# NOAA-GFDL/icebergs

Hardware: AMD Instinct MI355X
Metric: berg_steps_per_sec (higher is better)
Workload: dtype f64; 1 GPU; BASELINE configs[4] per-GPU share with configs[1] physics: 10000000 synthetic bergs/GPU (random mass classes), 360x200 lat-lon ocean grid, RK4 drag+Coriolis+melt+mass spreading, dt=1800 s, ignore_traj=T; bergs_per_gpu=10000000, grid=360x200, exchange=none (1 GPU), bergs_alive_at_end=9999583

## Files before the change

icebergs_amd/csrc/kid_cells.inc:

```
#include "kid_planes.hpp"

namespace {
struct GridPlanes { const double *st[KID_NGRID_STATIC]; const double *fo[KID_NFORCING]; };

__global__ void __launch_bounds__(256) pack_static_kernel(GridPlanes gp, GeoRec *geo, double *hotok, double *latref, double pi_180, int ni, int nj, int latlon, double Lx) {
  const int c = blockIdx.x * 256 + threadIdx.x;
  if (c >= ni * nj) return;
  GeoRec r;
  r.lon = gp.st[KID_G_LON][c]; r.lat = gp.st[KID_G_LAT][c]; r.area = gp.st[KID_G_AREA][c]; r.msk = gp.st[KID_G_MSK][c];
  geo[c] = r;
  if (latref) { double s_, c_; sincos(r.lat * pi_180, &s_, &c_); latref[2 * c] = s_; latref[2 * c + 1] = c_; }
  const int il = c % ni, jl = c / ni;
  double ok = 0.;
  if (il >= 1 && jl >= 1 && il + 1 < ni && jl + 1 < nj) {
    const double *lon = gp.st[KID_G_LON], *lat = gp.st[KID_G_LAT];
    const double x0 = lon[c - ni - 1], y0 = lat[c - ni - 1];
    const double x1 = mod_around(lon[c - ni], x0, Lx), y1 = lat[c - ni];
    const double x2 = mod_around(lon[c], x0, Lx), y2 = lat[c];
    const double x3 = mod_around(lon[c - 1], x0, Lx), y3 = lat[c - 1];
    const double k0 = (x1 - x0) * (y2 - y1) - (y1 - y0) * (x2 - x1), k1 = (x2 - x1) * (y3 - y2) - (y2 - y1) * (x3 - x2);
    const double k2 = (x3 - x2) * (y0 - y3) - (y3 - y2) * (x0 - x3), k3 = (x0 - x3) * (y1 - y0) - (y0 - y3) * (x1 - x0);
    const bool convex = (k0 > 0. && k1 > 0. && k2 > 0. && k3 > 0.) || (k0 < 0. && k1 < 0. && k2 < 0. && k3 < 0.);
    const bool polar = latlon && dmax(dmax(y0, y1), dmax(y2, y3)) >= 89.999;
    const double *lo = gp.st[KID_G_LON];
    const bool rect = lo[c - 1] == lo[c - ni - 1] && lo[c] == lo[c - ni] && lat[c - ni] == lat[c - ni - 1] && lat[c] == lat[c - 1];
    if (convex && !polar) ok = rect ? 2. : 1.;
  }
  hotok[c] = ok;
}

enum { KID_PKT_CELLS_PER_WAVE = 32 };
__global__ void __launch_bounds__(256) pack_packets_kernel(const DevGrid g, double *__restrict__ pkt) {
  const int lane = (int)(threadIdx.x & 63), wave = (int)(threadIdx.x >> 6);
  const int j = (int)blockIdx.y;
  const int i0 = ((int)blockIdx.x * 4 + wave) * KID_PKT_CELLS_PER_WAVE;
  if (i0 >= g.ni) return;
  const bool second = lane < PK_SIZE - 64;
  const PacketSrc s0 = packet_source(g, lane), s1 = packet_source(g, second ? 64 + lane : 0);
  const bool row_inside = j >= 1 && j < g.nj - 1;
  const int i1 = min(i0 + KID_PKT_CELLS_PER_WAVE, g.ni);
  for (int ib = i0; ib < i1; ib += 8) {
    double a[8], a2[8];
#pragma unroll
    for (int u = 0; u < 8; ++u) {
      const int i = ib + u;
      const bool interior = row_inside && i >= 1 && i < g.ni - 1 && i < i1;
      const long long c = interior ? (long long)j * g.ni + i : (long long)g.ni + 1;
      a[u] = *reinterpret_cast<const double *>(s0.base + c * s0.stride);
      a2[u] = *reinterpret_cast<const double *>(s1.base + c * s1.stride);
    }
#pragma unroll
    for (int u = 0; u < 8; ++u) {
      const int i = ib + u;
      if (i >= i1) continue;
      const bool interior = row_inside && i >= 1 && i < g.ni - 1;
      const bool is_cos = lane < PK_CORNER && (lane & 7) == 0, is_sin = lane < PK_CORNER && (lane & 7) == 1;
      const bool rotated = __ballot((is_cos && a[u] != 1.) || (is_sin && a[u] != 0.)) != 0ull;
      const bool nan_stencil = __ballot(lane >= PK_DDX && lane < PK_AREA && a[u] != a[u]) != 0ull;
      double *o = pkt + ((long long)j * g.ni + i) * PK_GSTRIDE;
      o[lane] = interior ? a[u] : 0.;
      if (second) {
        double v = interior ? a2[u] : 0.;
        if (64 + lane == PK_HOTOK) v = interior ? ((v != 0. && !nan_stencil) ? 1. : -1.) * (1. + (v == 2. ? 2. : 0.) + (rotated ? 0. : 4.)) : 0.;
        o[64 + lane] = v;
      }
    }
  }
}

struct PrepExtras { double *ssh_copy; double *acc; int zero_planes; int *cnt0, *cnt1; };
__global__ void __launch_bounds__(256) pack_forcing_kernel(GridPlanes gp, VelRec *vel, TrcRec *trc, int ni, int nj, PrepExtras ex) {
  const int c = blockIdx.x * 256 + threadIdx.x;
  if (c >= ni * nj) return;
  if (ex.ssh_copy) ex.ssh_copy[c] = gp.fo[KID_F_SSH][c];
  if (ex.acc) {
    const size_t ncell = (size_t)ni * (size_t)nj;
    for (int q = 0; q < ex.zero_planes; ++q) ex.acc[(size_t)q * ncell + (size_t)c] = 0.;
  }
  if (c == 0) { if (ex.cnt0) *ex.cnt0 = 0; if (ex.cnt1) *ex.cnt1 = 0; }
  const int il = c % ni, jl = c / ni;
  VelRec v;
  v.cosr = gp.st[KID_G_COS][c]; v.sinr = gp.st[KID_G_SIN][c];
  v.uo = gp.fo[KID_F_UO][c]; v.vo = gp.fo[KID_F_VO][c]; v.ui = gp.fo[KID_F_UI][c]; v.vi = gp.fo[KID_F_VI][c];
  v.ua = gp.fo[KID_F_UA][c]; v.va = gp.fo[KID_F_VA][c];
  vel[c] = v;
  const double *dx = gp.st[KID_G_DX], *dy = gp.st[KID_G_DY], *msk = gp.st[KID_G_MSK], *ssh = gp.fo[KID_F_SSH];
  TrcRec t;
  t.sst = gp.fo[KID_F_SST][c]; t.sss = gp.fo[KID_F_SSS][c]; t.cn = gp.fo[KID_F_CN][c]; t.hi = gp.fo[KID_F_HI][c];
  t.od = gp.st[KID_G_OCEAN_DEPTH][c] + ssh[c];
  t.msk = msk[c];
  t.ddx = 0.; t.ddy = 0.;
  if (il + 1 < ni && jl >= 1) {
    const double dxp = 0.5 * (dx[c + 1] + dx[c + 1 - ni]);
    const double dx0 = 0.5 * (dx[c] + dx[c - ni]);
    t.ddx = 2. * (ssh[c + 1] - ssh[c]) / (dx0 + dxp) * msk[c + 1] * msk[c];
  }
  if (jl + 1 < nj && il >= 1) {
    const double dyp = 0.5 * (dy[c + ni] + dy[c + ni - 1]);
    const double dy0 = 0.5 * (dy[c] + dy[c - 1]);
    t.ddy = 2. * (ssh[c + ni] - ssh[c]) / (dy0 + dyp) * msk[c + ni] * msk[c];
  }
  trc[c] = t;
}

__global__ void set_grid_kernel(const DevGrid src, DevGrid *dst) { if (threadIdx.x == 0 && blockIdx.x == 0) *dst = src; }

__device__ __forceinline__ double nine_point(const DevGrid &g, const double *v, const size_t ncell, const int c, const int i, const bool wrap, const double a, const double m) {
  const int nic = g.iec - g.isc + 1, ni = g.ni;
  const int wm = (wrap && i == g.isc) ? nic : 0, wp = (wrap && i == g.iec) ? -nic : 0;
  double dmda = nine_point_sum([&](int di, int dj, int slot) { return v[(size_t)(slot - 1) * ncell + (size_t)(c + di + (di < 0 ? wm : (di > 0 ? wp : 0)) + dj * ni)]; });
  if (a > 0) dmda = dmda / a * m;
  return dmda;
}

__global__ void __launch_bounds__(256) gather_kernel(const DevGrid g, const kid_params p, double *__restrict__ acc,
                                                     double *__restrict__ out, const size_t ncell, double *__restrict__ totals,
                                                     const double *__restrict__ spread_mass_old, const double *__restrict__ spread_mass_tmp) {
  const int t = blockIdx.x * 256 + threadIdx.x;
  if (t < KID_NSCALAR) {
    totals[t] += (acc - KID_NSCALAR)[t];
    (acc - KID_NSCALAR)[t] = 0.;
  }
  const int nic = g.iec - g.isc + 1, njc = g.jec - g.jsc + 1;
  if (t >= nic * njc) return;
  const int i = g.isc + t % nic, j = g.jsc + t / nic;
  const int c = g.idx(i, j);
  const double a = g.geo[c].area, m = g.geo[c].msk;
  const int dm = p.diag_mask;
  const bool wrap = p.periodic_reentry != 0 && g.Lx > 0.;
  auto nine = [&](int base) { return nine_point(g, acc + (size_t)base * ncell, ncell, c, i, wrap, a, m); };
  double su = 0., sv = 0., sa = 0.;
  if ((dm & KID_DIAG_SPREAD_UVEL) || p.pass_fields_to_ocean_model) su = nine(KID_A_UVEL_ON_OCEAN);
  if ((dm & KID_DIAG_SPREAD_VVEL) || p.pass_fields_to_ocean_model) sv = nine(KID_A_VVEL_ON_OCEAN);
  if ((dm & KID_DIAG_SPREAD_AREA) || p.pass_fields_to_ocean_model) sa = dmin(nine(KID_A_AREA_ON_OCEAN), 1.0);
  const double sm = nine(KID_A_MASS_ON_OCEAN);
  out[(size_t)KID_O_SPREAD_MASS * ncell + c] = sm;
  out[(size_t)KID_O_SPREAD_AREA * ncell + c] = sa;
  out[(size_t)KID_O_SPREAD_UVEL * ncell + c] = su;
  out[(size_t)KID_O_SPREAD_VVEL * ncell + c] = sv;
  if ((dm & KID_DIAG_U_ICEBERG) || (dm & KID_DIAG_V_ICEBERG)) {
    const double mass = acc[(size_t)KID_A_MASS * ncell + c];
    if (dm & KID_DIAG_U_ICEBERG) acc[(size_t)KID_A_U_ICEBERG * ncell + c] = (mass > 0.) ? acc[(size_t)KID_A_U_ICEBERG * ncell + c] / mass : 0.;
    if (dm & KID_DIAG_V_ICEBERG) acc[(size_t)KID_A_V_ICEBERG * ncell + c] = (mass > 0.) ? acc[(size_t)KID_A_V_ICEBERG * ncell + c] / mass : 0.;
  }
  double ustar_h = 0.;
  if ((dm & KID_DIAG_USTAR_ICEBERG) || p.pass_fields_to_ocean_model) {
    const double du = su - g.vel[c].uo, dv = sv - g.vel[c].vo;
    const double dvo = sqrt(du * du + dv * dv);
    const double ustar = sqrt(p.cdrag_icebergs * (dvo * dvo + p.utide_icebergs * p.utide_icebergs));
    ustar_h = dmax(p.ustar_icebergs_bg, ustar);
    if (sa == 0.0) ustar_h = 0.;
  }
  out[(size_t)KID_O_USTAR_ICEBERG * ncell + c] = ustar_h;
  if (spread_mass_old)
    acc[(size_t)KID_A_FLOATING_MELT * ncell + c] = (a > 0.0) ? dmax((spread_mass_old[c] - (spread_mass_tmp ? spread_mass_tmp[c] : sm)) / p.dt, 0.0) : 0.0;
  if (p.apply_thickness_cutoff_to_gridded_melt && (p.melt_cutoff >= 0.) && (sa > 0.)) {
    const double ave_thickness = sm / (sa * p.rho_bergs);
    const double ave_draft = ave_thickness * (p.rho_bergs / RHO_SEAWATER);
    if ((g.ocean_depth[c] - ave_draft) < p.melt_cutoff) {
      acc[(size_t)KID_A_FLOATING_MELT * ncell + c] = 0.0; acc[(size_t)KID_A_CALVING_HFLX * ncell + c] = 0.0;
    }
  }
}

__global__ void __launch_bounds__(256) mass_gather_kernel(const DevGrid g, const double *__restrict__ acc, double *__restrict__ plane, const size_t ncell, const bool wrap) {
  const int t = blockIdx.x * 256 + threadIdx.x;
  const int nic = g.iec - g.isc + 1, njc = g.jec - g.jsc + 1;
  if (t >= nic * njc) return;
  const int i = g.isc + t % nic, j = g.jsc + t / nic;
  const int c = g.idx(i, j);
  plane[c] = nine_point(g, acc + (size_t)KID_A_MASS_ON_OCEAN * ncell, ncell, c, i, wrap, g.geo[c].area, g.geo[c].msk);
}

}

static DevGrid dev_grid(const kid_handle *h, int parity = -1) {
  const ForcingSet &fs = h->fset[parity < 0 ? h->forc_parity : parity];
  DevGrid g;
  g.isd = h->gd.isd; g.ied = h->gd.ied; g.jsd = h->gd.jsd; g.jed = h->gd.jed;
  g.isc = h->gd.isc; g.iec = h->gd.iec; g.jsc = h->gd.jsc; g.jec = h->gd.jec;
  g.ni = h->ni; g.nj = h->nj; g.latlon = h->gd.grid_is_latlon; g.regular = h->gd.grid_is_regular; g.Lx = h->gd.Lx;
  g.vel = fs.vel; g.trc = fs.trc; g.geo = h->d_geo; g.hotok = h->d_hotok; g.latref = h->d_latref;
  g.pkt = fs.pkt;
  g.dx = h->d_static[KID_G_DX]; g.dy = h->d_static[KID_G_DY]; g.ocean_depth = h->d_static[KID_G_OCEAN_DEPTH];
  g.ssh = h->d_forcing[KID_F_SSH];
  g.sin_lat_ref = sin((h->params.pi / 180.) * h->params.lat_ref);
  g.pi_180 = h->params.pi / 180.; g.r180_pi = 180. / h->params.pi; g.dydl = (180. / h->params.pi) / h->params.Rearth;
  g.rho_ratio = h->params.rho_bergs / RHO_SEAWATER;
  g.fl_e1 = exp(0.25 * h->params.pi);
  return g;
}
static bool footprint_needed(const kid_params &p) { return kid::footprint_needed(p.pass_fields_to_ocean_model, p.diag_mask); }
static int nacc_active(const kid_handle *h) { return kid::nacc_live(h->params.pass_fields_to_ocean_model, h->params.diag_mask); }
static double *on_ocean_base(const kid_handle *h) { return h->d_acc + (size_t)ON_OCEAN_ALL.first * h->ncell; }
static int zero_planes(kid_handle *h, const PlaneRange r) {
  KID_HIP(h, hipMemsetAsync(h->d_acc + (size_t)r.first * h->ncell, 0, (size_t)r.count * h->ncell * sizeof(double), h->stream));
  return KID_OK;
}
static int refuse(kid_handle *h, bool ok, const char *msg) { if (!ok) h->err = msg; return ok ? KID_OK : KID_EINVAL; }
static int need_static(kid_handle *h) { return refuse(h, h->forc.have_static, "kid_set_static_grid must be called first"); }
static int need_forcing(kid_handle *h) { return refuse(h, h->forc.have_forcing, "kid_set_forcing must be called before stepping"); }
static bool forcing_held(const kid_handle *h, int k) { return h->forc.held[k]; }
static GridPlanes grid_planes(const kid_handle *h, const double *const *src) {
  GridPlanes gp;
  for (int k = 0; k < KID_NGRID_STATIC; ++k) gp.st[k] = h->d_static[k];
  for (int k = 0; k < KID_NFORCING; ++k) gp.fo[k] = (src && src[k]) ? src[k] : h->d_forcing[k];
  return gp;
}

static int pack_packets(kid_handle *h) {
  const unsigned bx = (unsigned)((h->ni + 4 * KID_PKT_CELLS_PER_WAVE - 1) / (4 * KID_PKT_CELLS_PER_WAVE));
  hipLaunchKernelGGL(pack_packets_kernel, dim3(bx, (unsigned)h->nj), dim3(256), 0, h->stream, dev_grid(h), h->fset[h->forc_parity].pkt);
  KID_HIP(h, hipGetLastError());
  return KID_OK;
}
static int pack_static(kid_handle *h) {
  const int nb = (int)((h->ncell + 255) / 256);
  hipLaunchKernelGGL(pack_static_kernel, dim3(nb), dim3(256), 0, h->stream, grid_planes(h, nullptr), h->d_geo, h->d_hotok, h->d_latref, h->params.pi / 180., h->ni, h->nj, (int)h->gd.grid_is_latlon, h->gd.Lx);
  KID_HIP(h, hipGetLastError());
  return h->forc.have_forcing ? pack_packets(h) : KID_OK;
}
static const PrepExtras no_extras{nullptr, nullptr, 0, nullptr, nullptr};
static int pack_forcing(kid_handle *h, const double *const *src, const PrepExtras ex = no_extras) {
  const int nb = (int)((h->ncell + 255) / 256);
  if (h->side_mode == 2 || h->pipelined) h->forc_parity ^= 1;
  const ForcingSet &fs = h->fset[h->forc_parity];
  hipLaunchKernelGGL(pack_forcing_kernel, dim3(nb), dim3(256), 0, h->stream, grid_planes(h, src), fs.vel, fs.trc, h->ni, h->nj, ex);
  return pack_packets(h);
}
static int forcing_given(kid_handle *h, unsigned given, const double *const *src, bool sync, const PrepExtras ex = no_extras) {
  ForcingState &f = h->forc;
  const unsigned every = (1u << KID_NFORCING) - 1u;
  for (int k = 0; k < KID_NFORCING; ++k) f.held[k] = f.held[k] || ((given >> k) & 1u);
  f.have_planes = f.have_planes || (given & every) == every; f.have_forcing = true;
  const int rc = pack_forcing(h, src, ex);
  if (rc) return rc;
  if (sync) KID_HIP(h, hipStreamSynchronize(h->stream));
  return KID_OK;
}

static int launch_gather(kid_handle *h) {
  { const int rc_j = join_side(h); if (rc_j) return rc_j; }
  const DevGrid g = dev_grid(h);
  const int ncomp = (h->gd.iec - h->gd.isc + 1) * (h->gd.jec - h->gd.jsc + 1);
  hipLaunchKernelGGL(gather_kernel, dim3((unsigned)((ncomp + 255) / 256)), dim3(256), 0, h->stream, g, h->params, h->d_acc, h->d_out, h->ncell, h->d_totals,
                     (const double *)(h->params.find_melt_using_spread_mass ? h->d_spread_mass_old : nullptr),
                     (const double *)((h->params.find_melt_using_spread_mass && h->params.Iceberg_melt_without_decay) ? h->d_spread_mass_old + h->ncell : nullptr));
  KID_HIP(h, hipGetLastError());
  return KID_OK;
}
static int gather_mass_and_reset(kid_handle *h, double *dst) {
  const int ncomp = (h->gd.iec - h->gd.isc + 1) * (h->gd.jec - h->gd.jsc + 1);
  hipLaunchKernelGGL(mass_gather_kernel, dim3((unsigned)((ncomp + 255) / 256)), dim3(256), 0, h->stream, dev_grid(h), (const double *)h->d_acc, dst, h->ncell,
                     h->params.periodic_reentry != 0 && h->gd.Lx > 0.);
  return zero_planes(h, ON_OCEAN_ALL);
}

extern "C" {

int kid_set_static_grid(kid_handle *h, const double *const fields[KID_NGRID_STATIC]) {
  if (!h || !fields) return KID_EINVAL;
  KID_HIP(h, hipSetDevice(h->device));
  for (int k = 0; k < KID_NGRID_STATIC; ++k) {
    if (!fields[k]) { if (k == KID_G_LONC || k == KID_G_LATC) continue; h->err = "static grid field missing"; return KID_EINVAL; }
    KID_HIP(h, hipMemcpyAsync(h->d_static[k], fields[k], h->ncell * sizeof(double), hipMemcpyHostToDevice, h->stream));
  }
  h->forc.have_static = true; h->bond_ext_valid = false;
  h->forc.have_centres = fields[KID_G_LONC] && fields[KID_G_LATC];
  int rc = pack_static(h);
  if (!rc) rc = pack_forcing(h, nullptr);
  if (rc) return rc;
  KID_HIP(h, hipStreamSynchronize(h->stream));
  return KID_OK;
}
int kid_set_forcing(kid_handle *h, const double *const fields[KID_NFORCING]) {
  if (!h || !fields) return KID_EINVAL;
  if (need_static(h)) return KID_EINVAL;
  KID_HIP(h, hipSetDevice(h->device));
  unsigned given = 0u;
  for (int k = 0; k < KID_NFORCING; ++k) {
    if (!fields[k]) continue;
    KID_HIP(h, hipMemcpyAsync(h->d_forcing[k], fields[k], h->ncell * sizeof(double), hipMemcpyHostToDevice, h->stream));
    given |= 1u << k;
  }
  return forcing_given(h, given, nullptr, true);
}
int kid_set_forcing_device(kid_handle *h, const double *const fields[KID_NFORCING]) {
  if (!h || !fields) return KID_EINVAL;
  if (need_static(h)) return KID_EINVAL;
  KID_HIP(h, hipSetDevice(h->device));
  if (fields[KID_F_SSH]) KID_HIP(h, hipMemcpyAsync(h->d_forcing[KID_F_SSH], fields[KID_F_SSH], h->ncell * sizeof(double), hipMemcpyDeviceToDevice, h->stream));
  return forcing_given(h, fields[KID_F_SSH] ? 1u << KID_F_SSH : 0u, fields, false);
}
int kid_step_prepare(kid_handle *h, const double *const fields[KID_NFORCING]) {
  if (!h) return KID_EINVAL;
  if (need_static(h) || (!fields && need_forcing(h))) return KID_EINVAL;
  KID_HIP(h, hipSetDevice(h->device));
  h->redo_parity ^= 1;
  if (h->side_mode == 2) {
    h->redo_parity = h->lane_step & 1;
    if (h->evC_live) { KID_HIP(h, hipStreamWaitEvent(h->stream, h->evC, 0)); }
  }
  PrepExtras ex;
  ex.ssh_copy = (fields && fields[KID_F_SSH] && fields[KID_F_SSH] != h->d_forcing[KID_F_SSH]) ? h->d_forcing[KID_F_SSH] : nullptr;
  ex.acc = h->d_acc; ex.zero_planes = nacc_active(h);
  ex.cnt0 = h->d_redo_cnt[0][h->redo_parity]; ex.cnt1 = h->d_redo_cnt[1][h->redo_parity];
  const int rc = forcing_given(h, ex.ssh_copy ? 1u << KID_F_SSH : 0u, fields, false, ex);
  if (rc) return rc;
  h->acc_prezeroed = true; h->redo_prezeroed = true;
  return KID_OK;
}
int kid_zero_accumulators(kid_handle *h) {
  if (!h) return KID_EINVAL;
  KID_HIP(h, hipSetDevice(h->device));
  return zero_planes(h, PlaneRange{0, nacc_active(h)});
}
int kid_get_accumulators(kid_handle *h, double *acc, double *out, double *scalars) {
  if (!h) return KID_EINVAL;
  KID_HIP(h, hipSetDevice(h->device));
  { const int rc_j = join_side(h); if (rc_j) return rc_j; }
  if (acc) KID_HIP(h, hipMemcpyAsync(acc, h->d_acc, (size_t)KID_NACC * h->ncell * sizeof(double), hipMemcpyDeviceToHost, h->stream));
  if (out) KID_HIP(h, hipMemcpyAsync(out, h->d_out, (size_t)KID_NOUT * h->ncell * sizeof(double), hipMemcpyDeviceToHost, h->stream));
  if (scalars) KID_HIP(h, hipMemcpyAsync(scalars, h->d_totals, KID_NSCALAR * sizeof(double), hipMemcpyDeviceToHost, h->stream));
  KID_HIP(h, hipStreamSynchronize(h->stream));
  if (scalars) {
    int64_t alive = 0;
    int rc = kid_num_bergs(h, nullptr, &alive);
    if (rc) return rc;
    scalars[KID_S_NBERGS_ALIVE] = (double)alive;
  }
  return KID_OK;
}
int kid_accum_device_ptr(kid_handle *h, void **dev_ptr, int64_t *count) {
  if (!h || !dev_ptr || !count) return KID_EINVAL;
  *dev_ptr = h->d_acc - KID_NSCALAR;
  *count = (int64_t)((size_t)KID_NACC * h->ncell + KID_NSCALAR);
  return KID_OK;
}
int kid_accum_live_count(kid_handle *h, int64_t *count) {
  if (!h || !count) return KID_EINVAL;
  *count = (int64_t)((size_t)nacc_active(h) * h->ncell + KID_NSCALAR);
  return KID_OK;
}
int kid_bind_accum_buffer(kid_handle *h, void *dev_ptr, int64_t count) {
  if (!h) return KID_EINVAL;
  if (!dev_ptr) { h->d_acc = h->d_acc_own + KID_NSCALAR; h->acc_prezeroed = false; return KID_OK; }
  if (count < (int64_t)((size_t)KID_NACC * h->ncell + KID_NSCALAR)) { h->err = "accumulator buffer too small"; return KID_EINVAL; }
  h->d_acc = (double *)dev_ptr + KID_NSCALAR;
  h->acc_prezeroed = false;
  return KID_OK;
}
int kid_bind_spread_mass_old(kid_handle *h, void *dev_ptr, int64_t count) {
  if (!h) return KID_EINVAL;
  if (!dev_ptr) { h->d_spread_mass_old = h->d_spread_mass_old_own; return KID_OK; }
  if (count < (int64_t)(2 * h->ncell)) { h->err = "spread_mass_old buffer too small (2 planes)"; return KID_EINVAL; }
  h->d_spread_mass_old = (double *)dev_ptr;
  return KID_OK;
}

}
```

icebergs_amd/csrc/kid_handle.hpp:

```cpp
#pragma once
#include "kid_mem.hpp"

struct HipAllocator {
  static constexpr int unknown_error = (int)hipErrorInvalidValue;
  const hipStream_t *stream;
  int alloc(void **p, size_t bytes, kid::MemKind k) const { return (int)(k == kid::MEM_PINNED ? hipHostMalloc(p, bytes) : hipMalloc(p, bytes)); }
  int release(void *p, kid::MemKind k) const { return (int)(k == kid::MEM_PINNED ? hipHostFree(p) : hipFree(p)); }
  int fill(void *p, int byte, size_t bytes) const { return (int)hipMemsetAsync(p, byte, bytes, *stream); }
  int copy(void *dst, const void *src, size_t bytes) const { return (int)hipMemcpy(dst, src, bytes, hipMemcpyDeviceToDevice); }
};
struct Scratch { void *p = nullptr; size_t bytes = 0; };
struct HipMem : kid::MemOwner<HipAllocator> {
  explicit HipMem(const hipStream_t *stream) : kid::MemOwner<HipAllocator>(HipAllocator{stream}) {}
  template <class T> hipError_t dev(T *&p, size_t count, int fill = kid::MEM_NOFILL, kid::MemKind k = kid::MEM_DEVICE) { void *q = nullptr; const int e = alloc(&q, count * sizeof(T), k, fill); p = (T *)q; return (hipError_t)e; }
  template <class T> hipError_t pinned(T *&p, size_t count) { return dev(p, count, kid::MEM_NOFILL, kid::MEM_PINNED); }
  template <class T> hipError_t drop(T *&p) { void *q = p; const int e = release(&q); p = (T *)q; return (hipError_t)e; }
  template <class T> hipError_t regrow(T *&p, size_t keep_count, size_t count) { void *q = p; const int e = grow(&q, keep_count * sizeof(T), count * sizeof(T)); p = (T *)q; return (hipError_t)e; }
  hipError_t reserve(Scratch &t, size_t bytes) {
    if (t.p && t.bytes >= bytes) return hipSuccess;
    int e = release(&t.p);
    if (!e) e = alloc(&t.p, bytes, kid::MEM_DEVICE);
    t.bytes = e ? 0 : bytes;
    return (hipError_t)e;
  }
};

namespace {
enum { KID_PERM_MAX = KID_NB_F64 + KID_NB_I32 + 2 };
struct PermTable { const void *src[KID_PERM_MAX]; void *dst[KID_PERM_MAX]; int n8, n4; };
}

struct ForcingSet { VelRec *vel = nullptr; TrcRec *trc = nullptr; double *pkt = nullptr; DevGrid *d_grid = nullptr; };
struct ForcingState {
  bool have_static = false, have_forcing = false;
  bool have_centres = false;
  bool have_planes = false;
  bool held[KID_NFORCING] = {};
};

struct kid_handle {
  int device = 0;
  hipStream_t own_stream = nullptr, stream = nullptr;
  HipMem mem{&stream}, rp_mem{&stream};
  kid_grid_desc gd{};
  kid_params params{};
  int ni = 0, nj = 0;
  size_t ncell = 0;
  int64_t capacity = 0, n = 0;
  double auto_growth = 0.; int64_t auto_min_free = 0, auto_max_capacity = 0;
  double *d_static[KID_NGRID_STATIC] = {}, *d_forcing[KID_NFORCING] = {};
  GeoRec *d_geo = nullptr; double *d_hotok = nullptr; double *d_latref = nullptr;
  double *d_acc_own = nullptr, *d_acc = nullptr;
  double *d_out = nullptr;
  double *d_totals = nullptr;
  BergPtrs bp{};
  BergPtrs *d_bp = nullptr;
  kid_params *d_params = nullptr;
  bool tables_dirty = true;
  Scratch scan_tmp;
  unsigned long long *d_count = nullptr;
  int *d_redo_list = nullptr;
  hipStream_t side_stream = nullptr; bool pipelined = false;
  int *d_redo_list2 = nullptr, *d_redo_count2 = nullptr;
  int *d_redo_cnt[2][2] = {{nullptr, nullptr}, {nullptr, nullptr}};
  int redo_parity = 0; bool redo_prezeroed = false, acc_prezeroed = false;
  bool uploaded_nonzero[KID_NB_F64] = {};
  bool tail_valid = false;
  bool mig_mode = false;
  int32_t *d_keep = nullptr;
  long long mig_last[2] = {0, 0};
  long long halo_last[2] = {0, 0};
  bool halo_rows_live = false;
  bool env_ever_stored = false;
  bool env_off_requested = false;
  double *d_orient = nullptr;
  hipEvent_t evF[2] = {nullptr, nullptr}, evG[2] = {nullptr, nullptr}; bool evG_live[2] = {false, false};
  int side_mode = 0; int *d_lane = nullptr, *d_lane_alt = nullptr; hipEvent_t evR = nullptr; int lane_step = 1; bool lanes_active = false, carry_valid = false, evC_live = false;
  hipEvent_t evC = nullptr, evP = nullptr;
  ForcingSet fset[2]; int forc_parity = 0;
  struct DebugOpts { bool stable_resort = false, no_plain_build = false, fl_unfused = false, new_order_unfused = false, mts_always_label = false, mts_no_fused = false, rebin_eager = false, chksum_timing = false;
                     int mts_fused_blocks_cap = 0, mts_poll_limit = 0; } dbg;
  int32_t *d_iceberg_counter = nullptr;
  bool fl_place_warm = false;
  unsigned fl_step = 0;
  int *d_fl_cursor = nullptr;
  int *d_fl_promoted = nullptr;
  int32_t *d_fl_head = nullptr, *d_fl_next = nullptr; int64_t *d_fl_newid = nullptr; long long fl_ev_capacity = 0;
  unsigned *d_key[2] = {nullptr, nullptr}, *d_idx[2] = {nullptr, nullptr};
  Scratch sort_tmp;
  BergPtrs bp_alt{};
  bool rebin_pending = false;
  int64_t rebin_fused_count = 0;
  struct RebinPlan { PermTable t{}; int moved_f[KID_NB_F64] = {}; int nmf = 0; unsigned long long moved = 0ull; const unsigned *perm = nullptr; long long n = 0; } rplan;
  RebinTab *d_rb = nullptr;
  unsigned *d_cell_hist = nullptr; Scratch cscan_tmp; bool stable_resort = false;
  int resort_interval = 16, steps_since_sort = 0;
  MtsDev mts{}; MtsDev *d_mts = nullptr;
  int mb = 0; bool mts_ready = false, mts_dirty = true, have_bonds = false, visited = false;
  unsigned long long *d_key64[2] = {nullptr, nullptr}; int *d_rows[2] = {nullptr, nullptr};
  int *d_static_rows = nullptr; long long static_rows_n = -1, static_rows_cap = 0;
  unsigned long long *d_last_key = nullptr; int *d_order_flag = nullptr; long long order_n = -1;
  unsigned long long *d_bond_sig = nullptr; bool labels_stale = true;
  MtsDev mts_shadow{}; bool mts_shadow_valid = false;
  int conglom_batch = 8;
  Scratch mts_tmp;
  unsigned long long *d_bond_words = nullptr;
  double bond_ext[2] = {0., 0.}; bool bond_ext_valid = false;
  hipGraphExec_t sub_graph_exec = nullptr;
  long long sub_graph_n = -1; int sub_graph_steps = 0; bool sub_graph_pair = false; double sub_graph_dt = 0.; hipStream_t sub_graph_stream = nullptr;
  bool use_graph = true;
  int fused_blocks[2] = {0, 0};
  bool fused_ran = false;
  Flags flags{0, 0, 1, 0, 0};
  bool traj_on = false; kid_traj_params traj_params{}; double *d_traj_f[64] = {}; double *d_traj_day = nullptr; int64_t *d_traj_id = nullptr;
  int32_t *d_traj_year = nullptr, *d_traj_nbonds = nullptr; unsigned long long *d_traj_cursor = nullptr; long long traj_capacity = 0, traj_count_bound = 0; int traj_nf = 0;
  double *d_mig_buf = nullptr; long long mig_capacity = 0; unsigned long long *mig_word = nullptr;
  double *halo_buf = nullptr; long long halo_capacity = 0;
  double *d_btraj_f[16] = {}; int64_t *d_btraj_id[2] = {}; int32_t *d_btraj_i[2] = {}; long long btraj_capacity = 0, btraj_count_bound = 0;
  double *d_spread_mass_old = nullptr;
  double *d_spread_mass_old_own = nullptr;
  ForcingState forc;
  int restart_locate = 0;
  double *d_calv_state = nullptr, *d_calv_scal = nullptr, *d_calv_part = nullptr; unsigned char *d_calv_flag = nullptr; int2 *d_calv_list = nullptr; double *calv_host = nullptr; kid_calving_params calv_params{};
  bool calving_on = false, calving_first_call = true, rmean_init = false, rmean_hflx_init = false;
  double *d_ingest_stage = nullptr; size_t ingest_stage_count = 0; unsigned long long *d_ingest_key = nullptr;
  bool profile = false;
  hipEvent_t ev0 = nullptr, ev1 = nullptr, ev2 = nullptr, ev3 = nullptr;
  std::vector<std::pair<hipEvent_t, hipEvent_t>> pending;
  double berg_ms = 0., all_ms = 0.; int64_t berg_launches = 0;
  bool repro = false;
  struct Repro { double *stage = nullptr; int32_t *key = nullptr; unsigned long long *mask = nullptr; int *srows = nullptr; long long srows_n = -1;
                 unsigned long long *k64[2] = {nullptr, nullptr}; int *rows[2] = {nullptr, nullptr}; unsigned *k32[2] = {nullptr, nullptr};
                 int *cs = nullptr; double *cell_heat = nullptr, *part = nullptr; Scratch tmp; } rp;
  double *d_budget = nullptr, *d_budget_plane = nullptr;
  std::string err;
};

#define KID_HIP(h, call)                                                                      \
  do {                                                                                        \
    hipError_t e__ = (call);                                                                  \
    if (e__ != hipSuccess) {                                                                  \
      (h)->err = std::string(#call) + ": " + hipGetErrorString(e__);                          \
      return KID_EHIP;                                                                        \
    }                                                                                         \
  } while (0)

extern "C" {
static int refresh_tables(kid_handle *h), join_side(kid_handle *h);
static int rebin_flush(kid_handle *h);
static int rebin_plan(kid_handle *h, bool dead_last);
static int rebin_core(kid_handle *h, bool with_lane, int *list, const int *list_count), rebin_apply(kid_handle *h, bool with_lane, int *list, const int *list_count);
static bool plain_namelist(const kid_handle *h), lanes_eligible(const kid_handle *h);
static int repro_refuse(kid_handle *h);
static int mts_check_timeout(kid_handle *h), mts_fold_scalars(kid_handle *h);
static int halo_bergs_supported(kid_handle *h, const char *what);
static int auto_reserve(kid_handle *h, int64_t need, const char *what);
}
```

icebergs_amd/csrc/kid_hip.hip:

```cpp
#include <algorithm>
#include <chrono>
#include <cmath>
#include <cstdio>
#include <cstdlib>
#include <cstring>
#include <string.h>
#include <string>
#include <type_traits>
#include <utility>
#include <vector>
#include <unordered_map>
#include <hip/hip_runtime.h>
#include <rocprim/rocprim.hpp>
#include "../../include/kid.h"
#include "kid_device.hpp"
#include "kid_thermo.hpp"
#include "kid_footloose.hpp"
#include "kid_berg_kernel.hpp"
#include "kid_rows_plan.hpp"
#include "kid_fl_contact.hpp"
#include "kid_reserve_plan.hpp"

using namespace kid;

// ... 47 lines not shown
      h->err = "use_broken_bonds_for_substep_contact requires break_bonds_on_sub_steps, dem and iceberg_bonds_on (FW:1438-1447)"; return KID_EINVAL; }
    if (p->footloose) { h->err = "footloose together with mts is not implemented"; return KID_EUNSUPPORTED; }
  } else if (p->interactive_icebergs_on || p->iceberg_bonds_on) {
    if (p->Runge_not_Verlet) { h->err = "interacting / bonded bergs under the single-time-step scheme are implemented for Verlet only (Runge_not_Verlet=F)"; return KID_EUNSUPPORTED; }
    if (p->footloose && p->iceberg_bonds_on) { h->err = "footloose together with iceberg_bonds_on: bonded footloose calving (edge elements that calve, IB:2566-2585) is not implemented"; return KID_EUNSUPPORTED; }
    if (p->iceberg_bonds_on && !p->interactive_icebergs_on) { h->err = "iceberg_bonds_on without interactive_icebergs_on is not implemented"; return KID_EUNSUPPORTED; }
    if (p->max_bonds < 1 || p->max_bonds > KID_MAX_BONDS) { h->err = "max_bonds out of range"; return KID_EINVAL; }
  }
  if (p->tidal_drift > 0.) { h->err = "tidal_drift needs FMS's random stream: not supported"; return KID_EUNSUPPORTED; }
  if (p->find_melt_using_spread_mass && (p->mts || p->interactive_icebergs_on || p->footloose)) {
    h->err = "find_melt_using_spread_mass is implemented for the plain evolve loop only (no bonds, interactions or footloose)";
    return KID_EUNSUPPORTED;
  }
  if (p->Runge_not_Verlet && p->footloose) { h->err = "Runge_not_Verlet must be false to use footloose (FW:1485-1490)"; return KID_EINVAL; }
  if (p->footloose && !p->use_operator_splitting) { h->err = "use_operator_splitting must be true to use footloose (FW:1476)"; return KID_EINVAL; }
  return KID_OK;
}

extern "C" {

#ifndef KID_BUILD_ID
#define KID_BUILD_ID "unknown"
#endif
const char *kid_version(void) {
  return "kid_hip 0.3 (gfx950) src " KID_BUILD_ID
#ifdef KID_EXACT_MATH
         " exact-math"
#endif
#ifdef KID_EXPERIMENTS
         " EXPERIMENTS"
#endif
      ;
}
int64_t kid_sizeof(int which) {
  switch (which) { case 0: return (int64_t)sizeof(kid_params); case 1: return (int64_t)sizeof(kid_grid_desc);
                   case 2: return (int64_t)sizeof(kid_berg_soa); case 3: return (int64_t)sizeof(kid_bond_soa);
                   case 4: return (int64_t)sizeof(kid_forcing_in);
                   case 5: return (int64_t)sizeof(kid_calving_params); case 6: return (int64_t)sizeof(kid_calving_in); default: return -1; }
}
#ifdef KID_EXP_TIMING
int kid_exp_timing(unsigned long long *out, int reset) {
  if (out) {
    std::vector<unsigned long long> all((size_t)KID_TPROF_WAVES * 16);
    if (hipMemcpyFromSymbol(all.data(), HIP_SYMBOL(kid_tprof), all.size() * sizeof(unsigned long long)) != hipSuccess) return KID_EHIP;
    for (int q = 0; q < 16; ++q) out[q] = 0ull;
    for (size_t r = 0; r < (size_t)KID_TPROF_WAVES; ++r) for (int q = 0; q < 16; ++q) out[q] += all[r * 16 + q];
  }
  if (reset) {
    void *sym = nullptr;
    if (hipGetSymbolAddress(&sym, HIP_SYMBOL(kid_tprof)) != hipSuccess || hipMemset(sym, 0, (size_t)KID_TPROF_WAVES * 16 * sizeof(unsigned long long)) != hipSuccess) return KID_EHIP;
  }
  return KID_OK;
}
#endif
static thread_local std::string destroy_err;
const char *kid_last_error(const kid_handle *h) { return h ? h->err.c_str() : destroy_err.empty() ? "null handle" : destroy_err.c_str(); }

int kid_create(const kid_grid_desc *grid, const kid_params *params, int64_t capacity, int device, kid_handle **out) {
  if (!grid || !params || !out || capacity <= 0) return KID_EINVAL;
  if (capacity > (int64_t(1) << 29)) return KID_EINVAL;
  int ndev = 0;
  if (hipGetDeviceCount(&ndev) != hipSuccess || ndev <= 0) return KID_ENODEV;
  if (device < 0 || device >= ndev) return KID_ENODEV;
  kid_handle *h = new kid_handle();
  *out = h;
  h->device = device;
  KID_HIP(h, hipSetDevice(device));
  h->gd = *grid;
  h->ni = grid->ied - grid->isd + 1; h->nj = grid->jed - grid->jsd + 1;
  if (h->ni < 5 || h->nj < 5 || grid->isc - grid->isd < 2 || grid->ied - grid->iec < 2 || grid->jsc - grid->jsd < 2 || grid->jed - grid->jec < 2) {
    h->err = "grid needs a halo of at least 2 cells"; return KID_EINVAL;
  }
  h->ncell = (size_t)h->ni * (size_t)h->nj;
  int rc = check_params(h, params);
  if (rc) return rc;
  h->params = *params;
  h->flags.footprint = footprint_needed(h->params) ? 1 : 0;
  h->capacity = capacity;
  if (getenv("KID_MTS_NO_GRAPH")) h->use_graph = false;
  h->dbg.stable_resort = getenv("KID_STABLE_RESORT") != nullptr; h->dbg.no_plain_build = getenv("KID_NO_PLAIN_BUILD") != nullptr;
  h->dbg.fl_unfused = getenv("KID_FL_UNFUSED") != nullptr; h->dbg.new_order_unfused = getenv("KID_NEW_ORDER_UNFUSED") != nullptr;
  h->dbg.rebin_eager = getenv("KID_REBIN_EAGER") != nullptr; h->dbg.chksum_timing = getenv("KID_CHKSUM_TIMING") != nullptr;
  h->dbg.mts_always_label = getenv("KID_MTS_ALWAYS_LABEL") != nullptr; h->dbg.mts_no_fused = getenv("KID_MTS_NO_FUSED") != nullptr;
  if (const char *e = getenv("KID_MTS_FUSED_BLOCKS_CAP")) h->dbg.mts_fused_blocks_cap = atoi(e);
  if (const char *e = getenv("KID_MTS_POLL_LIMIT")) h->dbg.mts_poll_limit = atoi(e);
  KID_HIP(h, hipStreamCreateWithFlags(&h->own_stream, hipStreamNonBlocking));
  h->stream = h->own_stream;
  const size_t cap = (size_t)capacity;
  for (auto &plane : h->d_static) KID_HIP(h, h->mem.dev(plane, h->ncell, 0));
  for (auto &plane : h->d_forcing) KID_HIP(h, h->mem.dev(plane, h->ncell, 0));
  for (ForcingSet &fs : h->fset) {
    KID_HIP(h, h->mem.dev(fs.vel, h->ncell)); KID_HIP(h, h->mem.dev(fs.trc, h->ncell)); KID_HIP(h, h->mem.dev(fs.d_grid, 1));
    KID_HIP(h, h->mem.dev(fs.pkt, h->ncell * PK_GSTRIDE, 0));
  }
  KID_HIP(h, h->mem.dev(h->d_geo, h->ncell));
  KID_HIP(h, h->mem.dev(h->d_hotok, h->ncell, 0));
  if (grid->grid_is_latlon) KID_HIP(h, h->mem.dev(h->d_latref, 2 * h->ncell));
  KID_HIP(h, h->mem.dev(h->d_acc_own, (size_t)KID_NACC * h->ncell + KID_NSCALAR, 0));
  h->d_acc = h->d_acc_own + KID_NSCALAR;
  KID_HIP(h, h->mem.dev(h->d_out, (size_t)KID_NOUT * h->ncell, 0));
  KID_HIP(h, h->mem.dev(h->d_totals, KID_NSCALAR, 0));
  for (auto &field : h->bp.f) KID_HIP(h, h->mem.dev(field, cap, 0));
  for (auto &field : h->bp.i) KID_HIP(h, h->mem.dev(field, cap, 0));
  KID_HIP(h, h->mem.dev(h->bp.id, cap, 0));
  KID_HIP(h, h->mem.dev(h->d_bp, 1));
  KID_HIP(h, h->mem.dev(h->d_rb, 1));
  KID_HIP(h, h->mem.dev(h->d_params, 1));
  KID_HIP(h, h->mem.dev(h->d_lane, cap, 0));
  KID_HIP(h, h->mem.dev(h->d_count, 4));
  KID_HIP(h, h->mem.dev(h->d_iceberg_counter, h->ncell, 0));
  KID_HIP(h, h->mem.dev(h->d_fl_cursor, 1));
  for (int **q : {&h->d_redo_list, &h->d_redo_list2}) KID_HIP(h, h->mem.dev(*q, cap));
  KID_HIP(h, h->mem.dev(h->d_redo_count2, 4, 0));
  for (int part = 0; part < 2; ++part) for (int par = 0; par < 2; ++par) h->d_redo_cnt[part][par] = h->d_redo_count2 + (2 * part + par);
  for (hipEvent_t *e : {&h->evC, &h->evP, &h->evF[0], &h->evF[1], &h->evG[0], &h->evG[1]}) KID_HIP(h, hipEventCreateWithFlags(e, hipEventDisableTiming));
  for (hipEvent_t *e : {&h->ev0, &h->ev1, &h->ev2, &h->ev3}) KID_HIP(h, hipEventCreate(e));
  KID_HIP(h, hipStreamSynchronize(h->stream));
  return KID_OK;
}

int kid_destroy(kid_handle *h) {
  if (!h) return KID_EINVAL;
  (void)hipSetDevice(h->device);
  (void)hipDeviceSynchronize();
  if (h->sub_graph_exec) (void)hipGraphExecDestroy(h->sub_graph_exec);
  for (hipEvent_t e : {h->evR, h->evC, h->evP, h->evF[0], h->evF[1], h->evG[0], h->evG[1], h->ev0, h->ev1, h->ev2, h->ev3}) if (e) (void)hipEventDestroy(e);
  for (auto &pe : h->pending) { (void)hipEventDestroy(pe.first); (void)hipEventDestroy(pe.second); }
  if (h->own_stream) (void)hipStreamDestroy(h->own_stream);
  const int e_rp = h->rp_mem.free_all(), e_mem = h->mem.free_all();
  const hipError_t e = (hipError_t)(e_rp ? e_rp : e_mem);
  delete h;
  if (e == hipSuccess) return KID_OK;
  destroy_err = std::string("kid_destroy: freeing the handle's memory: ") + hipGetErrorString(e);
  return KID_EHIP;
}

int kid_memory_in_use(int64_t *device_bytes, int64_t *pinned_bytes) {
  if (device_bytes) *device_bytes = kid::mem_in_use(kid::MEM_DEVICE).load();
  if (pinned_bytes) *pinned_bytes = kid::mem_in_use(kid::MEM_PINNED).load();
  return KID_OK;
}

int kid_set_params(kid_handle *h, const kid_params *params) {
  if (!h || !params) return KID_EINVAL;
  int rc = check_params(h, params);
  if (rc) return rc;
  if (!h->tables_dirty && h->d_params) {
    kid_params a = h->params, b = *params;
    a.current_year = b.current_year = 0; a.current_yearday = b.current_yearday = 0.;
    if (std::memcmp(&a, &b, sizeof(kid_params)) == 0) {
      h->params = *params;
      KID_HIP(h, hipSetDevice(h->device));
      hipLaunchKernelGGL(set_time_kernel, dim3(1), dim3(64), 0, h->stream, params->current_year, params->current_yearday, h->d_params);
      KID_HIP(h, hipGetLastError());
      return KID_OK;
    }
  }
  h->params = *params;
  h->tables_dirty = true;
  h->labels_stale = true;
  h->flags.footprint = footprint_needed(h->params) ? 1 : 0;
  if (!h->params.old_interp_flds_order && !h->env_off_requested) h->flags.store_env = 1;
  return KID_OK;
}
static int join_side(kid_handle *h) {
  for (int q = 0; q < 2; ++q)
// ... 259 lines not shown
```

Before: 11.85 billion berg-steps/s.

## Fuse forcing pack and packet build into one LDS-tiled prepass kernel

Replaces the two-kernel pipeline (pack_forcing_kernel writing vel/trc records, then pack_packets_kernel re-reading them to build per-cell neighbourhood packets) with a single tiled kernel. Each block stages a 32x4 tile plus a one-cell halo of vel/trc/geo/hotok values in shared memory, writes the vel/trc records, and assembles the packets from LDS. Block-to-tile mapping is remapped so neighbouring tiles land on the same XCD. This removes one launch and a global round trip of the record arrays, at the cost of halo recomputation and extra LDS use. The old path stays behind an env flag, and a readback API is added for checking results.

Result: no change. 11.95 billion berg-steps/s, median of 6 (+0.9%).

```diff
diff --git a/icebergs_amd/csrc/kid_cells.inc b/icebergs_amd/csrc/kid_cells.inc
--- a/icebergs_amd/csrc/kid_cells.inc
+++ b/icebergs_amd/csrc/kid_cells.inc
@@ -1,4 +1,5 @@
 #include "kid_planes.hpp"
+#include "kid_prepass_tile.hpp"
 
 namespace {
 struct GridPlanes { const double *st[KID_NGRID_STATIC]; const double *fo[KID_NFORCING]; };
@@ -103,6 +104,114 @@
   trc[c] = t;
 }
 
+static_assert(PK_CORNER == kid::PQ_CORNER && PK_T0 == kid::PQ_T0 && PK_DDX == kid::PQ_DDX && PK_DDY == kid::PQ_DDY && PK_AREA == kid::PQ_AREA &&
+              PK_MSK == kid::PQ_MSK && PK_HOTOK == kid::PQ_HOTOK && PK_SIZE == kid::PQ_SIZE && PK_SIZE <= 128, "packet_ref is packet_source in cell offsets");
+static_assert(sizeof(VelRec) == 64 && sizeof(TrcRec) == 64 && sizeof(GeoRec) == 32 && kid::PT_TRC == 8 && kid::PT_GEO == 16 && kid::PT_HOTOK == 20, "slot layout");
+template <int TX, int TY, int NT>
+__global__ void __launch_bounds__(NT) prepass_fused_kernel(GridPlanes gp, VelRec *__restrict__ vel, TrcRec *__restrict__ trc, const GeoRec *__restrict__ geo,
+                                                           const double *__restrict__ hotok, double *__restrict__ pkt, int ni, int nj, PrepExtras ex) {
+  constexpr kid::PrepassTile T{TX, TY, NT};
+  __shared__ double slot[T.slots() * kid::PT_SLOT];
+  const kid::TileOrigin o = kid::prepass_origin(T, (int)blockIdx.x, ni, nj);
+  if (blockIdx.x == 0 && threadIdx.x == 0) { if (ex.cnt0) *ex.cnt0 = 0; if (ex.cnt1) *ex.cnt1 = 0; }
+  if (ex.acc) {
+    const size_t ncell = (size_t)ni * (size_t)nj;
+    for (int k = (int)threadIdx.x; k < T.cells(); k += NT) {
+      const int il = o.i0 + k % TX, jl = o.j0 + k / TX;
+      if (!kid::cell_exists(il, jl, ni, nj)) continue;
+      for (int q = 0; q < ex.zero_planes; ++q) ex.acc[(size_t)q * ncell + (size_t)(jl * ni + il)] = 0.;
+    }
+  }
+  for (int s = (int)threadIdx.x; s < T.slots(); s += NT) {
+    const int li = kid::prepass_slot_li(T, s), lj = kid::prepass_slot_lj(T, s);
+    const int il = o.i0 + li, jl = o.j0 + lj;
+    if (!kid::cell_exists(il, jl, ni, nj)) continue;
+    const int c = jl * ni + il;
+    const double *dx = gp.st[KID_G_DX], *dy = gp.st[KID_G_DY], *msk = gp.st[KID_G_MSK], *ssh = gp.fo[KID_F_SSH];
+    VelRec v;
+    v.cosr = gp.st[KID_G_COS][c]; v.sinr = gp.st[KID_G_SIN][c];
+    v.uo = gp.fo[KID_F_UO][c]; v.vo = gp.fo[KID_F_VO][c]; v.ui = gp.fo[KID_F_UI][c]; v.vi = gp.fo[KID_F_VI][c];
+    v.ua = gp.fo[KID_F_UA][c]; v.va = gp.fo[KID_F_VA][c];
+    TrcRec t;
+    t.sst = gp.fo[KID_F_SST][c]; t.sss = gp.fo[KID_F_SSS][c]; t.cn = gp.fo[KID_F_CN][c]; t.hi = gp.fo[KID_F_HI][c];
+    t.od = gp.st[KID_G_OCEAN_DEPTH][c] + ssh[c];
+    t.msk = msk[c];
+    const bool hx = kid::ddx_defined(il, jl, ni, nj), hy = kid::ddy_defined(il, jl, ni, nj);
+    const int xe = hx ? c + 1 : c, xs = hx ? c - ni : c, xse = hx ? c + 1 - ni : c;
+    const int yn = hy ? c + ni : c, yw = hy ? c - 1 : c, ynw = hy ? c + ni - 1 : c;
+    const double dx_c = dx[c], dx_e = dx[xe], dx_se = dx[xse], dx_s = dx[xs], dy_c = dy[c], dy_n = dy[yn], dy_nw = dy[ynw], dy_w = dy[yw];
+    const double ssh_c = ssh[c], ssh_e = ssh[xe], ssh_n = ssh[yn], msk_e = msk[xe], msk_n = msk[yn];
+    const GeoRec r = geo[c];
+    const double ok = hotok[c];
+    {
+      const double dxp = 0.5 * (dx_e + dx_se);
+      const double dx0 = 0.5 * (dx_c + dx_s);
+      const double ddx = 2. * (ssh_e - ssh_c) / (dx0 + dxp) * msk_e * t.msk;
+      t.ddx = hx ? ddx : 0.;
+    }
+    {
+      const double dyp = 0.5 * (dy_n + dy_nw);
+      const double dy0 = 0.5 * (dy_c + dy_w);
+      const double ddy = 2. * (ssh_n - ssh_c) / (dy0 + dyp) * msk_n * t.msk;
+      t.ddy = hy ? ddy : 0.;
+    }
+    double *d = slot + s * kid::PT_SLOT;
+    d[kid::PT_VEL + 0] = v.cosr; d[kid::PT_VEL + 1] = v.sinr; d[kid::PT_VEL + 2] = v.uo; d[kid::PT_VEL + 3] = v.vo;
+    d[kid::PT_VEL + 4] = v.ui; d[kid::PT_VEL + 5] = v.vi; d[kid::PT_VEL + 6] = v.ua; d[kid::PT_VEL + 7] = v.va;
+    d[kid::PT_TRC + 0] = t.sst; d[kid::PT_TRC + 1] = t.sss; d[kid::PT_TRC + 2] = t.cn; d[kid::PT_TRC + 3] = t.hi;
+    d[kid::PT_TRC + 4] = t.od; d[kid::PT_TRC + 5] = t.ddx; d[kid::PT_TRC + 6] = t.ddy; d[kid::PT_TRC + 7] = t.msk;
+    d[kid::PT_GEO + 0] = r.lon; d[kid::PT_GEO + 1] = r.lat; d[kid::PT_GEO + 2] = r.area; d[kid::PT_GEO + 3] = r.msk;
+    d[kid::PT_HOTOK] = ok;
+    if (ex.ssh_copy && kid::prepass_owned(T, li, lj)) ex.ssh_copy[c] = ssh_c;
+  }
+  __syncthreads();
+  {
+    double *const rec[2] = {reinterpret_cast<double *>(vel), reinterpret_cast<double *>(trc)};
+    for (int e = (int)threadIdx.x; e < T.cells() * 8; e += NT) {
+      const int k = e >> 3, f = e & 7, li = k % TX, lj = k / TX;
+      const int il = o.i0 + li, jl = o.j0 + lj;
+      if (!kid::cell_exists(il, jl, ni, nj)) continue;
+      const double *d = slot + kid::prepass_slot(T, li, lj) * kid::PT_SLOT;
+      const size_t at = (size_t)(jl * ni + il) * 8 + (size_t)f;
+      rec[0][at] = d[kid::PT_VEL + f];
+      rec[1][at] = d[kid::PT_TRC + f];
+    }
+  }
+  const int lane = (int)(threadIdx.x & 63), wave = __builtin_amdgcn_readfirstlane((int)(threadIdx.x >> 6));
+  const bool second = lane < PK_SIZE - 64;
+  const int src0 = kid::packet_lds_index(T, 0, 0, lane), src1 = kid::packet_lds_index(T, 0, 0, second ? 64 + lane : 0);
+  const bool is_cos = lane < PK_CORNER && (lane & 7) == 0, is_sin = lane < PK_CORNER && (lane & 7) == 1;
+  constexpr int U = 4;
+  for (int k0 = wave * U; k0 < T.cells(); k0 += (NT / 64) * U) {
+    double a[U], a2[U];
+#pragma unroll
+    for (int u = 0; u < U; ++u) {
+      const int k = k0 + u, li = k % TX, lj = k / TX;
+      const bool interior = k < T.cells() && kid::cell_has_neighbourhood(o.i0 + li, o.j0 + lj, ni, nj);
+      const int at = interior ? kid::prepass_slot(T, li, lj) * kid::PT_SLOT - kid::prepass_slot(T, 0, 0) * kid::PT_SLOT : 0;
+      const double x = slot[at + src0], x2 = slot[at + src1];
+      a[u] = interior ? x : 0.;
+      a2[u] = interior ? x2 : 0.;
+    }
+#pragma unroll
+    for (int u = 0; u < U; ++u) {
+      const int k = k0 + u, li = k % TX, lj = k / TX;
+      const int i = o.i0 + li, j = o.j0 + lj;
+      if (k >= T.cells() || !kid::cell_exists(i, j, ni, nj)) continue;
+      const bool interior = kid::cell_has_neighbourhood(i, j, ni, nj);
+      const bool rotated = __ballot((is_cos && a[u] != 1.) || (is_sin && a[u] != 0.)) != 0ull;
+      const bool nan_stencil = __ballot(lane >= PK_DDX && lane < PK_AREA && a[u] != a[u]) != 0ull;
+      double *out = pkt + ((long long)j * ni + i) * PK_GSTRIDE;
+      out[lane] = a[u];
+      if (second) {
+        double w = a2[u];
+        if (64 + lane == PK_HOTOK) w = interior ? ((w != 0. && !nan_stencil) ? 1. : -1.) * (1. + (w == 2. ? 2. : 0.) + (rotated ? 0. : 4.)) : 0.;
+        out[64 + lane] = w;
+      }
+    }
+  }
+}
+
 __global__ void set_grid_kernel(const DevGrid src, DevGrid *dst) { if (threadIdx.x == 0 && blockIdx.x == 0) *dst = src; }
 
 __device__ __forceinline__ double nine_point(const DevGrid &g, const double *v, const size_t ncell, const int c, const int i, const bool wrap, const double a, const double m) {
@@ -225,8 +334,15 @@
   const int nb = (int)((h->ncell + 255) / 256);
   if (h->side_mode == 2 || h->pipelined) h->forc_parity ^= 1;
   const ForcingSet &fs = h->fset[h->forc_parity];
-  hipLaunchKernelGGL(pack_forcing_kernel, dim3(nb), dim3(256), 0, h->stream, grid_planes(h, src), fs.vel, fs.trc, h->ni, h->nj, ex);
-  return pack_packets(h);
+  if (h->dbg.prepass_unfused) {
+    hipLaunchKernelGGL(pack_forcing_kernel, dim3(nb), dim3(256), 0, h->stream, grid_planes(h, src), fs.vel, fs.trc, h->ni, h->nj, ex);
+    return pack_packets(h);
+  }
+  constexpr kid::PrepassTile T = kid::PREPASS_TILE;
+  hipLaunchKernelGGL((prepass_fused_kernel<T.tx, T.ty, T.threads>), dim3((unsigned)kid::prepass_blocks(T, h->ni, h->nj)), dim3((unsigned)T.threads), 0, h->stream,
+                     grid_planes(h, src), fs.vel, fs.trc, (const GeoRec *)h->d_geo, (const double *)h->d_hotok, fs.pkt, h->ni, h->nj, ex);
+  KID_HIP(h, hipGetLastError());
+  return KID_OK;
 }
 static int forcing_given(kid_handle *h, unsigned given, const double *const *src, bool sync, const PrepExtras ex = no_extras) {
   ForcingState &f = h->forc;
@@ -308,6 +424,18 @@
   const int rc = forcing_given(h, ex.ssh_copy ? 1u << KID_F_SSH : 0u, fields, false, ex);
   if (rc) return rc;
   h->acc_prezeroed = true; h->redo_prezeroed = true;
+  return KID_OK;
+}
+int kid_prepass_readback(kid_handle *h, int parity, double *vel, double *trc, double *pkt, int *parity_out) {
+  if (!h || parity < -1 || parity > 1) return KID_EINVAL;
+  KID_HIP(h, hipSetDevice(h->device));
+  { const int rc_j = join_side(h); if (rc_j) return rc_j; }
+  const ForcingSet &fs = h->fset[parity < 0 ? h->forc_parity : parity];
+  if (vel) KID_HIP(h, hipMemcpyAsync(vel, fs.vel, h->ncell * sizeof(VelRec), hipMemcpyDeviceToHost, h->stream));
+  if (trc) KID_HIP(h, hipMemcpyAsync(trc, fs.trc, h->ncell * sizeof(TrcRec), hipMemcpyDeviceToHost, h->stream));
+  if (pkt) KID_HIP(h, hipMemcpyAsync(pkt, fs.pkt, h->ncell * PK_GSTRIDE * sizeof(double), hipMemcpyDeviceToHost, h->stream));
+  KID_HIP(h, hipStreamSynchronize(h->stream));
+  if (parity_out) *parity_out = h->forc_parity;
   return KID_OK;
 }
 int kid_zero_accumulators(kid_handle *h) {
diff --git a/icebergs_amd/csrc/kid_handle.hpp b/icebergs_amd/csrc/kid_handle.hpp
--- a/icebergs_amd/csrc/kid_handle.hpp
+++ b/icebergs_amd/csrc/kid_handle.hpp
@@ -78,7 +78,7 @@
   int side_mode = 0; int *d_lane = nullptr, *d_lane_alt = nullptr; hipEvent_t evR = nullptr; int lane_step = 1; bool lanes_active = false, carry_valid = false, evC_live = false;
   hipEvent_t evC = nullptr, evP = nullptr;
   ForcingSet fset[2]; int forc_parity = 0;
-  struct DebugOpts { bool stable_resort = false, no_plain_build = false, fl_unfused = false, new_order_unfused = false, mts_always_label = false, mts_no_fused = false, rebin_eager = false, chksum_timing = false;
+  struct DebugOpts { bool stable_resort = false, no_plain_build = false, fl_unfused = false, new_order_unfused = false, mts_always_label = false, mts_no_fused = false, rebin_eager = false, chksum_timing = false, prepass_unfused = false;
                      int mts_fused_blocks_cap = 0, mts_poll_limit = 0; } dbg;
   int32_t *d_iceberg_counter = nullptr;
   bool fl_place_warm = false;
diff --git a/icebergs_amd/csrc/kid_hip.hip b/icebergs_amd/csrc/kid_hip.hip
--- a/icebergs_amd/csrc/kid_hip.hip
+++ b/icebergs_amd/csrc/kid_hip.hip
@@ -153,6 +153,7 @@
   h->dbg.fl_unfused = getenv("KID_FL_UNFUSED") != nullptr; h->dbg.new_order_unfused = getenv("KID_NEW_ORDER_UNFUSED") != nullptr;
   h->dbg.rebin_eager = getenv("KID_REBIN_EAGER") != nullptr; h->dbg.chksum_timing = getenv("KID_CHKSUM_TIMING") != nullptr;
   h->dbg.mts_always_label = getenv("KID_MTS_ALWAYS_LABEL") != nullptr; h->dbg.mts_no_fused = getenv("KID_MTS_NO_FUSED") != nullptr;
+  h->dbg.prepass_unfused = getenv("KID_PREPASS_UNFUSED") != nullptr;
   if (const char *e = getenv("KID_MTS_FUSED_BLOCKS_CAP")) h->dbg.mts_fused_blocks_cap = atoi(e);
   if (const char *e = getenv("KID_MTS_POLL_LIMIT")) h->dbg.mts_poll_limit = atoi(e);
   KID_HIP(h, hipStreamCreateWithFlags(&h->own_stream, hipStreamNonBlocking));
diff --git a/icebergs_amd/csrc/kid_prepass_tile.hpp b/icebergs_amd/csrc/kid_prepass_tile.hpp
--- /dev/null
+++ b/icebergs_amd/csrc/kid_prepass_tile.hpp
@@ -0,0 +1,56 @@
+#pragma once
+
+namespace kid {
+
+struct PrepassTile {
+  int tx, ty;
+  int threads;
+  constexpr int width() const { return tx + 2; }
+  constexpr int slots() const { return (tx + 2) * (ty + 2); }
+  constexpr int cells() const { return tx * ty; }
+};
+constexpr PrepassTile PREPASS_TILE{32, 4, 256};
+
+enum { PT_VEL = 0, PT_TRC = 8, PT_GEO = 16, PT_HOTOK = 20, PT_SLOT = 21 };
+
+constexpr int prepass_tiles_x(const PrepassTile t, int ni) { return (ni + t.tx - 1) / t.tx; }
+constexpr int prepass_tiles_y(const PrepassTile t, int nj) { return (nj + t.ty - 1) / t.ty; }
+constexpr int prepass_blocks(const PrepassTile t, int ni, int nj) { return prepass_tiles_x(t, ni) * prepass_tiles_y(t, nj); }
+
+constexpr int PREPASS_XCDS = 8;
+constexpr int prepass_tile_of_block(int block, int nblocks) {
+  const int q = nblocks / PREPASS_XCDS, r = nblocks % PREPASS_XCDS, die = block % PREPASS_XCDS;
+  return (die < r ? die * (q + 1) : r * (q + 1) + (die - r) * q) + block / PREPASS_XCDS;
+}
+struct TileOrigin { int i0, j0; };
+constexpr TileOrigin prepass_origin(const PrepassTile t, int block, int ni, int nj) {
+  const int tile = prepass_tile_of_block(block, prepass_blocks(t, ni, nj));
+  return {(tile % prepass_tiles_x(t, ni)) * t.tx, (tile / prepass_tiles_x(t, ni)) * t.ty};
+}
+constexpr int prepass_slot(const PrepassTile t, int li, int lj) { return (lj + 1) * t.width() + (li + 1); }
+constexpr int prepass_slot_li(const PrepassTile t, int slot) { return slot % t.width() - 1; }
+constexpr int prepass_slot_lj(const PrepassTile t, int slot) { return slot / t.width() - 1; }
+constexpr bool prepass_owned(const PrepassTile t, int li, int lj) { return li >= 0 && li < t.tx && lj >= 0 && lj < t.ty; }
+
+constexpr bool cell_exists(int i, int j, int ni, int nj) { return i >= 0 && i < ni && j >= 0 && j < nj; }
+constexpr bool cell_has_neighbourhood(int i, int j, int ni, int nj) { return i >= 1 && i + 1 < ni && j >= 1 && j + 1 < nj; }
+constexpr bool ddx_defined(int i, int j, int ni, int ) { return i + 1 < ni && j >= 1; }
+constexpr bool ddy_defined(int i, int j, int , int nj) { return j + 1 < nj && i >= 1; }
+
+struct PacketRef { int rec, field, di, dj; };
+enum { PQ_CORNER = 32, PQ_T0 = 40, PQ_DDX = 45, PQ_DDY = 51, PQ_AREA = 57, PQ_MSK = 58, PQ_HOTOK = 67, PQ_SIZE = 68 };
+constexpr PacketRef packet_ref(int q) {
+  if (q < PQ_CORNER) return {PT_VEL, q & 7, -(((q >> 3) & 1) ? 0 : 1), -(((q >> 3) & 2) ? 0 : 1)};
+  if (q < PQ_T0) return {PT_GEO, (q - PQ_CORNER) & 1, -((((q - PQ_CORNER) >> 1) & 1) ? 0 : 1), -((((q - PQ_CORNER) >> 1) & 2) ? 0 : 1)};
+  if (q < PQ_DDX) return {PT_TRC, q - PQ_T0, 0, 0};
+  if (q < PQ_DDY) return {PT_TRC, 5, -((q - PQ_DDX) / 3), 1 - (q - PQ_DDX) % 3};
+  if (q < PQ_AREA) return {PT_TRC, 6, 1 - (q - PQ_DDY) % 3, -((q - PQ_DDY) / 3)};
+  if (q == PQ_AREA) return {PT_GEO, 2, 0, 0};
+  if (q < PQ_HOTOK) return {PT_GEO, 3, (q - PQ_MSK) % 3 - 1, (q - PQ_MSK) / 3 - 1};
+  return {PT_HOTOK, 0, 0, 0};
+}
+constexpr int packet_lds_index(const PrepassTile t, int li, int lj, int q) {
+  return prepass_slot(t, li + packet_ref(q).di, lj + packet_ref(q).dj) * PT_SLOT + packet_ref(q).rec + packet_ref(q).field;
+}
+
+}
```
